# mazouziwissem/improving_yolov8_CBAM_SwinBlock

Hardware: AMD Instinct MI355X
Metric: images/sec fwd+bwd YOLOv8s-CBAM-Swin bs=32 640x640 (higher is better)
Workload: dtype bf16; 1 GPU; yolov8s.yaml (nc=1) forward + v8 loss + backward + clip + SGD-nesterov + EMA step, bs=32/GPU 640x640 (CBAM + 2x SwinBlock + SPPF5 + SPPF7); global_batch=32, imgsz=640, parallelism=dp1

## Files before the change

improving_yolov8_cbam_swinblock_amd/csrc/common.h:

```cpp
#pragma once
#include <hip/hip_runtime.h>
#include <stdint.h>
#include <stdio.h>

#include <type_traits>

#include "../../include/ymi.h"

typedef __bf16 bf16_t;
typedef __attribute__((ext_vector_type(8))) __bf16 bf16x8;
typedef __attribute__((ext_vector_type(4))) __bf16 bf16x4;
typedef __attribute__((ext_vector_type(4))) float f32x4;
typedef __attribute__((ext_vector_type(2))) float f32x2;
typedef __attribute__((ext_vector_type(4))) uint32_t u32x4;
typedef __attribute__((ext_vector_type(2))) uint32_t u32x2;

typedef const __attribute__((address_space(1))) void* gptr_t;
typedef __attribute__((address_space(3))) void* lptr_t;

#define YMI_WAVE 64

void ymi_set_error(const char* fmt, ...);
#define YMI_CHECK_ARG(cond, ...)          \
    do {                                  \
// ... 29 lines not shown
static inline bool ymi_same_shape(const ymi_tensor* a, const ymi_tensor* b) {
    return a->n == b->n && a->h == b->h && a->w == b->w && a->c == b->c;
}
enum YmiOpt {
    OPT_EW_PPT,
    OPT_EW_CAP,
    OPT_RED_CAP,
    OPT_XCD_SHIFT,
    OPT_ATTN_TILED,
    OPT_WGRAD_BLOCKS,
    OPT_WGRAD_BLOCKS128,
    OPT_IGEMM_TILE_BM,
    OPT_IGEMM_TILE_BN,
    OPT_BN_TAIL,
    OPT_WGRAD_PATCH,
    OPT_COUNT
};
int ymi_opt(int id);
static inline int ew_ppt() { return ymi_opt(OPT_EW_PPT); }
static inline int ew_cap() { return ymi_opt(OPT_EW_CAP); }
static inline int64_t ew_capped(int64_t gb) {
    if (gb > ew_cap()) gb = ew_cap();
    return (gb + 7) / 8 * 8;
}
static inline int64_t ew_blocks(int64_t P, int rows) {
    int64_t gb = (P + (int64_t)rows * ew_ppt() - 1) / ((int64_t)rows * ew_ppt());
    if (gb < 1024) gb = (P + rows - 1) / rows < 1024 ? (P + rows - 1) / rows : 1024;
    return ew_capped(gb);
}
template <typename T> struct TypeTag {
    typedef T type;
};
template <int ACT> using ActTag = std::integral_constant<int, ACT>;
// ... 411 lines not shown
```

improving_yolov8_cbam_swinblock_amd/csrc/runtime.hip:

```cpp
#include <stdarg.h>
#include <string.h>

#include <stdlib.h>

#include "common.h"

static thread_local char g_err[512] = "";

void ymi_set_error(const char* fmt, ...) {
    va_list ap;
    va_start(ap, fmt);
    vsnprintf(g_err, sizeof(g_err), fmt, ap);
    va_end(ap);
}

extern "C" int ymi_version(void) { return YMI_VERSION; }
extern "C" const char* ymi_last_error(void) { return g_err; }

__device__ __attribute__((aligned(256))) unsigned char ymi_zero_page_storage[256];

const void* ymi_zero_page() {
    static thread_local int cached_dev = -1;
    static thread_local void* cached_ptr = nullptr;
    int dev = 0;
// ... 1 lines not shown
    if (dev != cached_dev) {
        void* p = nullptr;
        if (hipGetSymbolAddress(&p, HIP_SYMBOL(ymi_zero_page_storage)) != hipSuccess) return nullptr;
        cached_ptr = p;
        cached_dev = dev;
    }
    return cached_ptr;
}

struct OptEntry {
    const char* name;
    int value;
};
static OptEntry g_opts[OPT_COUNT] = {
    {"ew_ppt", 64}, {"ew_cap", 512}, {"red_cap", 512}, {"xcd_shift", 0}, {"attn_tiled", 0}, {"wgrad_blocks", 1280}, {"wgrad_blocks128", 768},
    {"igemm_tile_bm", 0}, {"igemm_tile_bn", 0}, {"bn_tail", 0}, {"wgrad_patch", 1},
};
static void opts_from_env() {
    for (int i = 0; i < OPT_COUNT; ++i) {
        char env[64] = "YMI_";
        size_t n = 4;
        for (const char* c = g_opts[i].name; *c && n + 1 < sizeof(env); ++c) env[n++] = (char)((*c >= 'a' && *c <= 'z') ? *c - 32 : *c);
        env[n] = 0;
        if (const char* v = getenv(env)) g_opts[i].value = atoi(v);
    }
    if (const char* t = getenv("YMI_IGEMM_TILE")) {
        int bm = 0, bn = 0;
        if (sscanf(t, "%d,%d", &bm, &bn) == 2) {
            g_opts[OPT_IGEMM_TILE_BM].value = bm;
            g_opts[OPT_IGEMM_TILE_BN].value = bn;
        }
    }
}
int ymi_opt(int id) {
    static const bool init = (opts_from_env(), true);
    (void)init;
    return g_opts[id].value;
}
extern "C" int ymi_set_option(const char* name, int64_t value) {
    (void)ymi_opt(0);
    for (int i = 0; name && i < OPT_COUNT; ++i)
        if (!strcmp(name, g_opts[i].name)) {
            g_opts[i].value = (int)value;
            return YMI_OK;
        }
    ymi_set_error("set_option: unknown option '%s'", name ? name : "(null)");
    return YMI_EINVAL;
}
extern "C" int64_t ymi_get_option(const char* name) {
    (void)ymi_opt(0);
    for (int i = 0; name && i < OPT_COUNT; ++i)
        if (!strcmp(name, g_opts[i].name)) return g_opts[i].value;
// ... 22 lines not shown
```

improving_yolov8_cbam_swinblock_amd/csrc/wgrad.hip:

```cpp
#include <stdlib.h>

#include <mutex>
#include <type_traits>

#include "common.h"

struct WgradArgs {
    const void* x;
    const void* dy;
    void* slab;
    int slab_bf16;
    float* bias_slab;
    const void* zero;
    int64_t ldx, ldy;
    int Mpix, H, W, Ho, Wo;
    int stride, pad, KW;
    int CoutP, Cin, NG;
    int pix_per_split;
    int nx, ny, splits, xcd_map;
    int pw_shift;
    uint32_t x_bytes, y_bytes;
    uint32_t wo_mul, wo_shr, ho_mul, ho_shr;
};

__device__ __forceinline__ int wg_fast_div(int n, uint32_t mul, uint32_t shr) { return (int)((__umulhi((uint32_t)n, mul) + (uint32_t)n) >> shr); }

constexpr int WG_BN = 128;
constexpr int WG_BK = 32;
constexpr int WG_NS = 2;
constexpr int WG_WAVES = 5;

template <typename T, int BM> constexpr size_t wgrad_lds_bytes() { return (size_t)WG_NS * WG_BK * (BM + WG_BN) * sizeof(T); }

__device__ __forceinline__ void wg_buffer_to_lds(const void* base, uint32_t bytes, lptr_t dst, uint32_t voff, uint32_t soff) {
#if defined(__HIP_DEVICE_COMPILE__)
    __builtin_amdgcn_raw_ptr_buffer_load_lds(__builtin_amdgcn_make_buffer_rsrc(const_cast<void*>(base), 0, bytes, 0x00020000), dst, 16, voff, soff, 0, 0);
#endif
}
__device__ __forceinline__ void wg_global_to_lds(const void* src, lptr_t dst) {
#if defined(__HIP_DEVICE_COMPILE__)
    __builtin_amdgcn_global_load_lds((gptr_t)src, dst, 16, 0, 0);
#endif
}
template <typename T> struct WFrag;

template <> struct WFrag<bf16_t> {
    static __device__ __forceinline__ void read2(bf16x8& f, const TrFragAddr& ad) {
        typedef __attribute__((ext_vector_type(2))) uint32_t u2;
        u2 lo, hi;
        asm volatile("ds_read_b64_tr_b16 %0, %1" : "=v"(lo) : "v"((uint32_t)(uintptr_t)ad.lo));
        asm volatile("ds_read_b64_tr_b16 %0, %1" : "=v"(hi) : "v"((uint32_t)(uintptr_t)ad.hi));
        const u32x4 v = {lo[0], lo[1], hi[0], hi[1]};
        f = __builtin_bit_cast(bf16x8, v);
    }
    template <int BM, int TR, int TC, bool BIAS>
    static __device__ __forceinline__ void step(const char* Ys, const char* Xs, int r0, int c0, int lane, f32x4 (&acc)[TR][TC], bool bias, f32x4 (&accb)[BIAS ? TR : 1]) {
        static_assert(WG_BK == 32, "one 32-deep sub-step");
        bf16x8 af[TR], bfr[TC];
        TrFragAddr ay[TR], ax[TC];
#pragma unroll
        for (int t = 0; t < TR; ++t) ay[t] = tr_frag_addr<tr_swz_mode(BM * 2)>(Ys, BM * 2, r0 + t * 16, lane);
#pragma unroll
        for (int t = 0; t < TC; ++t) ax[t] = tr_frag_addr<tr_swz_mode(WG_BN * 2)>(Xs, WG_BN * 2, c0 + t * 16, lane);
        __builtin_amdgcn_sched_barrier(0);
#pragma unroll
        for (int t = 0; t < TC; ++t) read2(bfr[t], ax[t]);
#pragma unroll
        for (int t = 0; t < TR; ++t) read2(af[t], ay[t]);
#pragma unroll
        for (int a = 0; a < TR; ++a) {
            __builtin_amdgcn_sched_barrier(0);
            if (a == 0) asm volatile("s_waitcnt lgkmcnt(%0)" ::"n"(2 * (TR - 1)) : "memory");
            else if (a == 1) asm volatile("s_waitcnt lgkmcnt(%0)" ::"n"(TR > 2 ? 2 * (TR - 2) : 0) : "memory");
            else if (a == 2) asm volatile("s_waitcnt lgkmcnt(%0)" ::"n"(TR > 3 ? 2 * (TR - 3) : 0) : "memory");
            else asm volatile("s_waitcnt lgkmcnt(0)" ::: "memory");
            asm volatile("" : "+v"(af[a]));
            if (a == 0) {
#pragma unroll
// ... 1 lines not shown
            }
#pragma unroll
            for (int b = 0; b < TC; ++b)
                acc[a][b] = __builtin_amdgcn_mfma_f32_16x16x32_bf16(bfr[b], af[a], acc[a][b], 0, 0, 0);
            if (BIAS && bias) {
                typedef __attribute__((ext_vector_type(8))) short s16x8;
                const s16x8 one8 = {0x3F80, 0x3F80, 0x3F80, 0x3F80, 0x3F80, 0x3F80, 0x3F80, 0x3F80};
                const bf16x8 ones = __builtin_bit_cast(bf16x8, one8);
                if constexpr (BIAS) accb[a] = __builtin_amdgcn_mfma_f32_16x16x32_bf16(ones, af[a], accb[a], 0, 0, 0);
            }
        }
        __builtin_amdgcn_sched_barrier(0);
    }
};
template <> struct WFrag<float> {
    template <int BM, int TR, int TC, bool BIAS>
    static __device__ __forceinline__ void step(const char* Ys, const char* Xs, int r0, int c0, int lane, f32x4 (&acc)[TR][TC], bool bias, f32x4 (&accb)[BIAS ? TR : 1]) {
        const int kq = lane >> 4, i = lane & 15;
#pragma unroll
        for (int ks = 0; ks < WG_BK / 4; ++ks) {
            float af[TR], bfr[TC];
#pragma unroll
            for (int t = 0; t < TR; ++t) af[t] = *reinterpret_cast<const float*>(Ys + ((4 * ks + kq) * BM + r0 + t * 16 + i) * 4);
#pragma unroll
            for (int t = 0; t < TC; ++t) bfr[t] = *reinterpret_cast<const float*>(Xs + ((4 * ks + kq) * WG_BN + c0 + t * 16 + i) * 4);
#pragma unroll
            for (int a = 0; a < TR; ++a)
#pragma unroll
                for (int b = 0; b < TC; ++b) acc[a][b] = __builtin_amdgcn_mfma_f32_16x16x4f32(bfr[b], af[a], acc[a][b], 0, 0, 0);
            if (BIAS && bias) {
#pragma unroll
                for (int a = 0; a < (BIAS ? TR : 1); ++a) accb[a] = __builtin_amdgcn_mfma_f32_16x16x4f32(1.0f, af[a], accb[a], 0, 0, 0);
            }
        }
    }
};

template <typename T, int BM> struct WgTile {
    static constexpr int NT = 256;
    static constexpr int CH = ElemTraits<T>::CH, ES = (int)sizeof(T);
    static constexpr int YCW = BM * ES / 16, XCW = WG_BN * ES / 16;
    static constexpr int YT = WG_BK * YCW < NT ? WG_BK * YCW : NT;
    static constexpr int NY = (WG_BK * YCW + NT - 1) / NT, NX = WG_BK * XCW / NT;
    static constexpr int WCOLS = WG_BN / 64, WROWS = (NT / 64) / WCOLS;
    static constexpr int WM = BM / WROWS, TR = WM / 16, TC = 4;
    static constexpr int YBYTES = WG_BK * BM * ES, XBYTES = WG_BK * WG_BN * ES, STAGE = YBYTES + XBYTES;
    static_assert(NY >= 1 && NX >= 1, "tile too small");
    static constexpr bool SWZ = std::is_same<T, bf16_t>::value;
    static_assert(NT / XCW >= 16 || !SWZ, "bf16: a block-wide load covers >= 16 rows, so a thread's rows share the row bits the swizzle uses");
    int yrow0, ych;
    bool y_cok, x_cok;
    int xrow0, ci, dh, dw;
    __device__ __forceinline__ WgTile(const WgradArgs& a, int tid, int j0, int co0) {
        const int ytid = tid % YT;
        yrow0 = ytid / YCW;
        const int ycc = SWZ ? ((ytid % YCW) ^ (tr_swz<tr_swz_mode(YCW * 16)>(yrow0) << 1)) : (ytid % YCW);
        ych = co0 + ycc * CH;
        y_cok = ych < a.CoutP;
        xrow0 = tid / XCW;
        const int xcc = SWZ ? ((tid % XCW) ^ (tr_swz<tr_swz_mode(XCW * 16)>(xrow0) << 1)) : (tid % XCW);
        const int j = j0 + xcc * CH;
        x_cok = j < a.NG;
        const int tap = x_cok ? j / a.Cin : 0;
        ci = x_cok ? j - tap * a.Cin : 0;
        dh = tap / a.KW - a.pad;
        dw = tap % a.KW - a.pad;
    }
    __device__ __forceinline__ int y_row(int i) const { return yrow0 + i * (NT / YCW); }
    __device__ __forceinline__ int x_row(int i) const { return xrow0 + i * (NT / XCW); }
    static __device__ __forceinline__ lptr_t y_slot(char* Ys, int i, int wave) { return (lptr_t)(Ys + (i * NT + (wave * 64) % YT) * 16); }
    static __device__ __forceinline__ lptr_t x_slot(char* Xs, int i, int wave) { return (lptr_t)(Xs + (i * NT + wave * 64) * 16); }
};

template <typename T, int BM> struct WgRasterWalk {
    using G = WgTile<T, BM>;
    const WgradArgs& a;
    const G& ld;
    const int wave, m_end;
    const int s_ = a.stride, ldx32 = (int)a.ldx, ldy32 = (int)a.ldy;
    const int q_ = WG_BK / a.Wo, r_ = WG_BK - q_ * a.Wo;
    const uint32_t d_step = (uint32_t)((q_ * s_ * a.W + r_ * s_) * ldx32);
    const uint32_t d_wwrap = (uint32_t)((s_ * a.W - a.Wo * s_) * ldx32);
    const uint32_t d_hwrap = (uint32_t)((a.H * a.W - a.Ho * s_ * a.W) * ldx32);
    const uint32_t y_step = (uint32_t)(WG_BK * ldy32);
    const int ws_lim = a.Wo * s_, hs_lim = a.Ho * s_;
    int x_ws[G::NX], x_hs[G::NX];
    uint32_t x_off[G::NX], y_off[G::NY];
    __device__ __forceinline__ WgRasterWalk(const WgradArgs& a_, const G& ld_, int wave_, int m_begin)
        : a(a_), ld(ld_), wave(wave_), m_end(min(a_.Mpix, m_begin + a_.pix_per_split)) {
#pragma unroll
        for (int i = 0; i < G::NX; ++i) {
            const int m = m_begin + ld.x_row(i);
            const int t = wg_fast_div(m, a.wo_mul, a.wo_shr);
            const int wo = m - t * a.Wo;
            const int n = wg_fast_div(t, a.ho_mul, a.ho_shr);
            const int ho = t - n * a.Ho;
            x_ws[i] = wo * s_;
            x_hs[i] = ho * s_;
            x_off[i] = (uint32_t)(((n * a.H + ho * s_ + ld.dh) * a.W + wo * s_ + ld.dw) * ldx32 + ld.ci);
        }
#pragma unroll
        for (int i = 0; i < G::NY; ++i) y_off[i] = (uint32_t)((m_begin + ld.y_row(i)) * ldy32 + ld.ych);
    }
    __device__ __forceinline__ void issue(char* Ys, int mk) {
        const T* __restrict__ xg = reinterpret_cast<const T*>(a.x);
        const T* __restrict__ yg = reinterpret_cast<const T*>(a.dy);
        const T* zero = reinterpret_cast<const T*>(a.zero);
        char* Xs = Ys + G::YBYTES;
        const int left = m_end - mk;
#pragma unroll
        for (int i = 0; i < G::NY; ++i) {
            const bool ok = ld.y_cok && ld.y_row(i) < left;
            const T* src = ok ? yg + y_off[i] : zero;
            wg_global_to_lds(src, ld.y_slot(Ys, i, wave));
            y_off[i] += y_step;
        }
#pragma unroll
        for (int i = 0; i < G::NX; ++i) {
            const bool ok = ld.x_cok && ld.x_row(i) < left && (unsigned)(x_hs[i] + ld.dh) < (unsigned)a.H && (unsigned)(x_ws[i] + ld.dw) < (unsigned)a.W;
            const T* src = ok ? xg + x_off[i] : zero;
            wg_global_to_lds(src, ld.x_slot(Xs, i, wave));
            x_ws[i] += r_ * s_;
            x_hs[i] += q_ * s_;
            x_off[i] += d_step;
            if (x_ws[i] >= ws_lim) {
                x_ws[i] -= ws_lim;
                x_hs[i] += s_;
                x_off[i] += d_wwrap;
            }
            while (x_hs[i] >= hs_lim) {
                x_hs[i] -= hs_lim;
                x_off[i] += d_hwrap;
            }
        }
    }
};

template <typename T, int BM> struct WgPatchWalk {
    using G = WgTile<T, BM>;
    static constexpr uint32_t OOR = 0x80000000u;
    static constexpr int ES = G::ES;
    const WgradArgs& a;
    const int wave;
    const int s_ = a.stride, ldx32 = (int)a.ldx, ldy32 = (int)a.ldy;
    const int pw = 1 << a.pw_shift, ph = WG_BK >> a.pw_shift;
    const uint32_t xbias = (uint32_t)((a.W + 1) * ldx32 * ES);
    uint32_t pvx[G::NX], pvy[G::NY];
    int pch[G::NX], pcw[G::NX];
    int p_wo, p_ho;
    uint32_t p_sx, p_sy;
    __device__ __forceinline__ WgPatchWalk(const WgradArgs& a_, const G& ld, int wave_, int m_begin) : a(a_), wave(wave_) {
#pragma unroll
        for (int i = 0; i < G::NX; ++i) {
            const int row = ld.x_row(i);
            const int pr = row >> a.pw_shift, pc = row & (pw - 1);
            pch[i] = pr * s_ + ld.dh;
            pcw[i] = pc * s_ + ld.dw;
            pvx[i] = ld.x_cok ? (uint32_t)(((pch[i] * a.W + pcw[i]) * ldx32 + ld.ci) * ES) + xbias : OOR;
        }
#pragma unroll
        for (int i = 0; i < G::NY; ++i) {
            const int row = ld.y_row(i);
            const int pr = row >> a.pw_shift, pc = row & (pw - 1);
            pvy[i] = ld.y_cok ? (uint32_t)(((pr * a.Wo + pc) * ldy32 + ld.ych) * ES) : OOR;
        }
        const int pidx = __builtin_amdgcn_readfirstlane(m_begin / WG_BK);
        const int npw = a.Wo >> a.pw_shift, nph = a.Ho / ph;
        const int t = pidx / npw, wp = pidx - t * npw;
        const int n = t / nph, hp = t - n * nph;
        p_wo = wp * pw;
        p_ho = hp * ph;
        p_sx = (uint32_t)(((n * a.H + p_ho * s_) * a.W + p_wo * s_) * ldx32 * ES);
        p_sy = (uint32_t)(((n * a.Ho + p_ho) * a.Wo + p_wo) * ldy32 * ES);
// ... 14 lines not shown
        p_sx += (uint32_t)(pw * s_ * ldx32 * ES);
        p_sy += (uint32_t)(pw * ldy32 * ES);
        if (p_wo == a.Wo) {
            p_wo = 0;
            p_ho += ph;
            p_sx += (uint32_t)((ph * s_ * a.W - a.Wo * s_) * ldx32 * ES);
            p_sy += (uint32_t)((ph * a.Wo - a.Wo) * ldy32 * ES);
            if (p_ho == a.Ho) {
                p_ho = 0;
                p_sx += (uint32_t)((a.H * a.W - a.Ho * s_ * a.W) * ldx32 * ES);
            }
        }
    }
};

template <typename S, int TR> struct SlabStage {
    static constexpr int ES = (int)sizeof(S);
    static constexpr int SROW = 64 * ES + 16;
    static constexpr int CPR = 64 * ES / 16;
    static constexpr int RPI = 64 / CPR;
    static constexpr int RP = TR < 4 / ES ? TR : 4 / ES;
    static constexpr int BYTES = RP * 16 * SROW;
    static_assert(TR % RP == 0, "whole passes");
};
template <typename S, int TR, int TC>
__device__ __forceinline__ void wg_store_slab_staged(char* ring, int wave, int lane, const f32x4 (&acc)[TR][TC], S* slab, int row0, int col0, int CoutP, int NG) {
    using St = SlabStage<S, TR>;
    constexpr int ES = St::ES, SROW = St::SROW, RP = St::RP;
    static_assert(TC * 16 == 64, "a wave's tile is 64 columns wide");
    __syncthreads();
    asm volatile("" : "+v"(lane));
    char* st = ring + wave * St::BYTES;
    const int l15 = lane & 15, l4 = lane >> 4;
    const int srow = lane / St::CPR, sch = lane % St::CPR;
    const int col = col0 + sch * (16 / ES);
#pragma unroll
    for (int r0 = 0; r0 < TR; r0 += RP) {
#pragma unroll
        for (int rr = 0; rr < RP; ++rr)
#pragma unroll
            for (int c = 0; c < TC; ++c) {
                char* p = st + (rr * 16 + l15) * SROW + (c * 16 + 4 * l4) * ES;
                if constexpr (std::is_same<S, float>::value) {
                    *reinterpret_cast<f32x4*>(p) = acc[r0 + rr][c];
                } else {
                    const bf16x4 v = {(bf16_t)acc[r0 + rr][c][0], (bf16_t)acc[r0 + rr][c][1], (bf16_t)acc[r0 + rr][c][2], (bf16_t)acc[r0 + rr][c][3]};
                    *reinterpret_cast<bf16x4*>(p) = v;
                }
            }
        __builtin_amdgcn_fence(__ATOMIC_RELEASE, "wavefront");
        __builtin_amdgcn_wave_barrier();
        __builtin_amdgcn_fence(__ATOMIC_ACQUIRE, "wavefront");
#pragma unroll
        for (int k = 0; k < RP * 16 / St::RPI; ++k) {
            const int row = k * St::RPI + srow;
            const u32x4 u = *reinterpret_cast<const u32x4*>(st + row * SROW + sch * 16);
            const int co = row0 + r0 * 16 + row;
            if (co < CoutP && col < NG) *reinterpret_cast<u32x4*>(slab + (int64_t)co * NG + col) = u;
        }
        __builtin_amdgcn_fence(__ATOMIC_RELEASE, "wavefront");
        __builtin_amdgcn_wave_barrier();
        __builtin_amdgcn_fence(__ATOMIC_ACQUIRE, "wavefront");
    }
}

template <typename T, int BM, bool BIAS, bool PATCH>
__global__ __launch_bounds__(256, (BM == 128 ? 3 : WG_WAVES)) void wgrad_kernel(WgradArgs a, BnRider rider) {
    using G = WgTile<T, BM>;
    constexpr int NT = G::NT, TR = G::TR, TC = G::TC, WM = G::WM, STAGE = G::STAGE, NS = WG_NS;
    constexpr int LDS = (int)wgrad_lds_bytes<T, BM>();
    static_assert(LDS == NS * STAGE, "the launcher's LDS bytes are the ring");
    static_assert(LDS >= (NT / 64) * SlabStage<bf16_t, TR>::BYTES && LDS >= (NT / 64) * SlabStage<float, TR>::BYTES, "the staged slab stores use the ring");
    static_assert(LDS >= BN_FINAL_RED * (int)sizeof(double), "a rider workgroup sums its slices in the ring");
    extern __shared__ __attribute__((aligned(16))) char smem[];

    const int tid = threadIdx.x, lane = tid & 63;
    const int wave = __builtin_amdgcn_readfirstlane(tid >> 6);
    const int wr = wave / G::WCOLS, wc = wave % G::WCOLS;
    int bx, by, bz;
    if (rider.nwg && (int)blockIdx.x < rider.nwg) {
        if ((int)blockIdx.x * 32 < rider.f.C) bn_final_block<NT, false>(rider.f, (int)blockIdx.x, reinterpret_cast<double*>(smem));
        return;
    }
    if (a.xcd_map) {
        const int id = (int)blockIdx.x - rider.nwg, xcd = id & 7, seq = id >> 3, nxy = a.nx * a.ny;
        const int zi = seq / nxy, t = seq - zi * nxy;
        const int spx = (a.splits + 7) >> 3;
        bz = xcd * spx + zi;
        if (zi >= spx || bz >= a.splits) return;
        by = t / a.nx;
        bx = t - by * a.nx;
    } else {
        bx = blockIdx.x; by = blockIdx.y; bz = blockIdx.z;
    }
    const int j0 = bx * WG_BN, co0 = by * BM;
    const int m_begin = bz * a.pix_per_split;
    const int m_end = min(a.Mpix, m_begin + a.pix_per_split);
    const G ld(a, tid, j0, co0);
    typename std::conditional<PATCH, WgPatchWalk<T, BM>, WgRasterWalk<T, BM>>::type walk(a, ld, wave, m_begin);

    f32x4 acc[TR][TC];
#pragma unroll
    for (int r = 0; r < TR; ++r)
#pragma unroll
        for (int c = 0; c < TC; ++c) acc[r][c] = f32x4{0.f, 0.f, 0.f, 0.f};

    const bool do_bias = BIAS && bx == 0 && wc == 0;
    f32x4 accb[BIAS ? TR : 1];
#pragma unroll
    for (int r = 0; r < (BIAS ? TR : 1); ++r) accb[r] = f32x4{0.f, 0.f, 0.f, 0.f};
    const int nk = (m_end - m_begin + WG_BK - 1) / WG_BK;
    constexpr int LPT = G::NY + G::NX;
#pragma unroll
    for (int s = 0; s < NS - 1; ++s)
        if (s < nk) walk.issue(smem + s * STAGE, m_begin + s * WG_BK);
    for (int kt = 0; kt < nk; ++kt) {
        if (kt + NS - 2 < nk) wait_vmcnt_barrier<LPT * (NS - 2)>();
        else wait_vmcnt_barrier<0>();
        if (kt + NS - 1 < nk) walk.issue(smem + ((kt + NS - 1) % NS) * STAGE, m_begin + (kt + NS - 1) * WG_BK);
        const char* Ys = smem + (kt % NS) * STAGE;
        WFrag<T>::template step<BM, TR, TC, BIAS>(Ys, Ys + G::YBYTES, wr * WM, wc * 64, lane, acc, do_bias, accb);
    }

    const int64_t slab_off = (int64_t)bz * a.CoutP * a.NG;
    const int row0 = co0 + wr * WM, col0 = j0 + wc * 64;
    const int l15 = lane & 15, l4 = lane >> 4;
    if (BIAS && do_bias && l4 == 0) {
#pragma unroll
        for (int r = 0; r < (BIAS ? TR : 1); ++r) {
            const int co = row0 + r * 16 + l15;
            if (co < a.CoutP) a.bias_slab[(int64_t)bz * a.CoutP + co] = accb[r][0];
        }
    }
    if constexpr (std::is_same<T, bf16_t>::value) {
        if (a.slab_bf16) wg_store_slab_staged<bf16_t>(smem, wave, lane, acc, reinterpret_cast<bf16_t*>(a.slab) + slab_off, row0, col0, a.CoutP, a.NG);
        else wg_store_slab_staged<float>(smem, wave, lane, acc, reinterpret_cast<float*>(a.slab) + slab_off, row0, col0, a.CoutP, a.NG);
    } else {
#pragma unroll
        for (int r = 0; r < TR; ++r) {
            const int co = row0 + r * 16 + l15;
// ... 98 lines not shown
        if (tab[mid].first_block <= (int)blockIdx.x) lo = mid;
        else hi = mid - 1;
    }
    const ymi_wgrad_pending e = tab[lo];
    if (e.slab_bf16) reduce_batch_body<true>(e, red);
    else reduce_batch_body<false>(e, red);
}

static void wg_find_divisor(int d, uint32_t* mul, uint32_t* shr) {
    int lg = 0;
    while ((1 << lg) < d) ++lg;
    *mul = (uint32_t)((((uint64_t)1 << 32) * (((uint64_t)1 << lg) - (uint64_t)d)) / (uint64_t)d + 1);
    *shr = (uint32_t)lg;
}

struct WgradPlan {
    int splits, pix_per_split;
    size_t slab_bytes;
};
static int wgrad_bm(int64_t coutp, bool bf16) {
    if (!bf16) return 64;
    if (coutp <= 32) return 32;
    return (coutp >= 128 && coutp % 128 == 0) || coutp >= 256 ? 128 : 64;
}
static WgradPlan wgrad_plan(int64_t mpix, int64_t coutp, int64_t ng, int bm, size_t slab_esize) {
    const int64_t tiles = ((ng + WG_BN - 1) / WG_BN) * ((coutp + bm - 1) / bm);
    const int target64 = ymi_opt(OPT_WGRAD_BLOCKS);
    const int target128 = ymi_opt(OPT_WGRAD_BLOCKS128);
    const int target = bm == 128 ? target128 : target64;
    int64_t s = (target + tiles - 1) / tiles;
    const int64_t smax = (mpix + 255) / 256;
    if (s > smax) s = smax;
    if (s < 1) s = 1;
    if (s >= 8) s = (s + 7) / 8 * 8 <= smax ? (s + 7) / 8 * 8 : s / 8 * 8;
    int64_t pps = (mpix + s - 1) / s;
    pps = (pps + WG_BK - 1) / WG_BK * WG_BK;
    s = (mpix + pps - 1) / pps;
    WgradPlan p;
    p.splits = (int)s;
    p.pix_per_split = (int)pps;
    p.slab_bytes = ((size_t)s * coutp * ng * slab_esize + 255) / 256 * 256;
    return p;
}

static int64_t pad_to(int64_t v, int64_t m) { return (v + m - 1) / m * m; }
constexpr int64_t WG_BIAS_ROWS = 2048 * 2 + 1;

extern "C" size_t ymi_conv2d_bwd_weight_workspace(int64_t m_rows, int64_t cout, int64_t cin, int64_t kh, int64_t kw) {
    const int64_t coutp = pad_to(cout, 8), cinp = pad_to(cin, 8);
    WgradPlan p = wgrad_plan(m_rows, coutp, kh * kw * cinp, 64, 4);
    const WgradPlan p128 = wgrad_plan(m_rows, coutp, kh * kw * cinp, 128, 4);
    if (p128.slab_bytes > p.slab_bytes) p = p128;
    return p.slab_bytes + (size_t)WG_BIAS_ROWS * coutp * sizeof(float) + 256;
}

static int wgrad_impl(const ymi_tensor* x, const ymi_tensor* dy, int64_t cout_real, int64_t cin_real, int64_t kh, int64_t kw, int64_t stride,
                      float* dw_oihw, float* dbias, void* workspace, size_t workspace_bytes, ymi_wgrad_pending* pending, void* stream);

struct WgradLaunch {
    WgradArgs a;
    dim3 grid;
    int bm;
    bool bf16;
    hipStream_t s;
    double flop, bytes;
};
template <typename T, int BM> static void wgrad_launch_tile(const WgradArgs& a, const BnRider& r, dim3 grid, hipStream_t s) {
    constexpr size_t lds = wgrad_lds_bytes<T, BM>();
    static_assert(lds <= 64 * 1024, "a larger ring needs hipFuncAttributeMaxDynamicSharedMemorySize");
    void (*kernel)(WgradArgs, BnRider) = a.bias_slab ? wgrad_kernel<T, BM, true, false> : wgrad_kernel<T, BM, false, false>;
    if constexpr (std::is_same<T, bf16_t>::value) {
        if (a.pw_shift >= 0) kernel = a.bias_slab ? wgrad_kernel<T, BM, true, true> : wgrad_kernel<T, BM, false, true>;
    }
    hipLaunchKernelGGL(kernel, grid, dim3(256), lds, s, a, r);
}
static void wgrad_launch(const WgradLaunch& h, const BnFinal* rider) {
    BnRider r{};
    dim3 grid = h.grid;
    if (rider && h.a.xcd_map) {
        r.f = *rider;
        r.nwg = ((rider->C + 31) / 32 + 7) / 8 * 8;
        grid.x += (unsigned)r.nwg;
    }
    int prof = -1;
    if (ymi_prof_enabled()) prof = ymi_prof_start(h.s, 1, h.flop, h.bytes, h.bf16 ? 2500.0 : 157.3);
    if (!h.bf16) wgrad_launch_tile<float, 64>(h.a, r, grid, h.s);
    else if (h.bm == 128) wgrad_launch_tile<bf16_t, 128>(h.a, r, grid, h.s);
    else if (h.bm == 32) wgrad_launch_tile<bf16_t, 32>(h.a, r, grid, h.s);
    else wgrad_launch_tile<bf16_t, 64>(h.a, r, grid, h.s);
    ymi_prof_stop(h.s, prof);
}
static struct WgradHeld {
    std::mutex mu;
    bool on = false;
    bool valid = false;
    WgradLaunch launch;
    int device = 0;
} g_held;
static int wgrad_current_device() {
    int d = 0;
    (void)hipGetDevice(&d);
// ... 83 lines not shown

static int wgrad_impl(const ymi_tensor* x, const ymi_tensor* dy, int64_t cout_real, int64_t cin_real, int64_t kh, int64_t kw, int64_t stride,
                      float* dw_oihw, float* dbias, void* workspace, size_t workspace_bytes, ymi_wgrad_pending* pending, void* stream) {
    YMI_CHECK_ARG(ymi_tensor_ok(x) && ymi_tensor_ok(dy) && dw_oihw && workspace, "conv2d_bwd_weight: bad argument");
    YMI_CHECK_ARG(x->dtype == dy->dtype, "conv2d_bwd_weight: dtype mismatch");
    const int ch = x->dtype == YMI_BF16 ? 8 : 4;
    YMI_CHECK_ARG(x->c % ch == 0 && x->ld % ch == 0 && dy->c % ch == 0 && dy->ld % ch == 0, "conv2d_bwd_weight: channels must be multiples of %d", ch);
    YMI_CHECK_ARG(kh == kw && (kh == 1 || kh == 3) && (stride == 1 || stride == 2), "conv2d_bwd_weight: k in {1,3}, stride in {1,2}");
    const int64_t pad = kh / 2;
    YMI_CHECK_ARG(dy->n == x->n && dy->h == (x->h + 2 * pad - kh) / stride + 1 && dy->w == (x->w + 2 * pad - kw) / stride + 1, "conv2d_bwd_weight: shapes");
    YMI_CHECK_ARG(cout_real <= dy->c && cin_real <= x->c, "conv2d_bwd_weight: real channel counts");
    YMI_CHECK_ARG(ymi_pixels(x) * x->ld < (1ll << 31) && ymi_pixels(dy) * dy->ld < (1ll << 31), "conv2d_bwd_weight: too large");
    const int64_t mpix = ymi_pixels(dy);
    const int64_t ng = kh * kw * x->c;
    const bool bf16 = x->dtype == YMI_BF16;
    const int bm = wgrad_bm(dy->c, bf16), bn = WG_BN;
    WgradPlan p = wgrad_plan(mpix, dy->c, ng, bm, bf16 ? 2 : 4);
    const bool slab_bf16 = bf16 && p.splits >= 16;
    if (bf16 && !slab_bf16) p = wgrad_plan(mpix, dy->c, ng, bm, 4);
    size_t need = p.slab_bytes + (dbias ? (size_t)WG_BIAS_ROWS * dy->c * sizeof(float) : 0);
    if (workspace_bytes < need) {
        ymi_set_error("conv2d_bwd_weight: workspace %zu < %zu bytes", workspace_bytes, need);
        return YMI_EWORKSPACE;
    }
    WgradArgs a{};
    a.x = x->data; a.dy = dy->data; a.slab = workspace; a.slab_bf16 = slab_bf16 ? 1 : 0; a.zero = ymi_zero_page();
    a.bias_slab = dbias ? reinterpret_cast<float*>(reinterpret_cast<char*>(workspace) + p.slab_bytes) : nullptr;
    YMI_CHECK_ARG(!dbias || p.splits <= WG_BIAS_ROWS, "conv2d_bwd_weight: too many splits for the bias partials");
    a.ldx = x->ld; a.ldy = dy->ld;
    a.Mpix = (int)mpix; a.H = (int)x->h; a.W = (int)x->w; a.Ho = (int)dy->h; a.Wo = (int)dy->w;
    a.stride = (int)stride; a.pad = (int)pad; a.KW = (int)kw;
    a.CoutP = (int)dy->c; a.Cin = (int)x->c; a.NG = (int)ng; a.pix_per_split = p.pix_per_split;
    wg_find_divisor(a.Wo, &a.wo_mul, &a.wo_shr);
    wg_find_divisor(a.Ho, &a.ho_mul, &a.ho_shr);
// ... 7 lines not shown
                const int pw = 1 << sh, ph = WG_BK >> sh;
                if (dy->w % pw == 0 && dy->h % ph == 0) {
                    a.pw_shift = sh;
                    break;
                }
            }
            a.x_bytes = (uint32_t)xb;
            a.y_bytes = (uint32_t)yb;
        }
    }
    a.xcd_map = p.splits >= 8 ? 1 : 0;
    dim3 grid((unsigned)a.nx, (unsigned)a.ny, (unsigned)p.splits);
    if (a.xcd_map) grid = dim3((unsigned)(8 * ((p.splits + 7) / 8) * a.nx * a.ny), 1, 1);
    hipStream_t s = (hipStream_t)stream;
    const double es = (double)ymi_esize(x->dtype);
    WgradLaunch h{a, grid, bm, bf16, s, 2.0 * (double)mpix * (double)dy->c * (double)ng,
                  ((double)ymi_pixels(x) * x->c + (double)mpix * dy->c) * es + (double)dy->c * ng * 4.0};
    {
        std::lock_guard<std::mutex> lk(g_held.mu);
        wgrad_flush_held_locked();
        if (pending && g_held.on && a.xcd_map) {
            g_held.launch = h;
            g_held.device = wgrad_current_device();
            g_held.valid = true;
        } else {
            wgrad_launch(h, nullptr);
        }
    }
    YMI_CHECK_LAUNCH("wgrad");
    if (pending) {
        *pending = ymi_wgrad_record(a.slab, dw_oihw, (int64_t)a.CoutP * a.NG, p.splits, a.NG, a.Cin, (int)cout_real, (int)cin_real, (int)(kh * kw), slab_bf16,
// ... 16 lines not shown
```

Baseline: 2791 images/sec.

## Add shape-matched wgrad tile widths for narrow 1x1 and 3x3 Cin=32 convs

Adds two new bf16 weight-gradient tile forms: a 64-wide N tile for 1x1 convs with at most 64 input channels, and a 288-wide tile built from nine 32-channel tap sub-images for 3x3 convs with Cin=32. This avoids wasted MFMA work and padded loads when the reduction dimension (taps*Cin) does not fill 128-column tiles. The change brings a wide-tile MFMA step with grouped LDS reads, generalised slab staging, and occupancy-aware split planning. The risks are more register and LDS pressure for the 288 tile and more template instantiations.

```diff
diff --git a/improving_yolov8_cbam_swinblock_amd/csrc/common.h b/improving_yolov8_cbam_swinblock_amd/csrc/common.h
--- a/improving_yolov8_cbam_swinblock_amd/csrc/common.h
+++ b/improving_yolov8_cbam_swinblock_amd/csrc/common.h
@@ -67,9 +67,12 @@
     OPT_IGEMM_TILE_BN,
     OPT_BN_TAIL,
     OPT_WGRAD_PATCH,
+    OPT_WGRAD_BN,
+    OPT_WGRAD_BN_LAST,
     OPT_COUNT
 };
 int ymi_opt(int id);
+void ymi_opt_store(int id, int value);
 static inline int ew_ppt() { return ymi_opt(OPT_EW_PPT); }
 static inline int ew_cap() { return ymi_opt(OPT_EW_CAP); }
 static inline int64_t ew_capped(int64_t gb) {
diff --git a/improving_yolov8_cbam_swinblock_amd/csrc/runtime.hip b/improving_yolov8_cbam_swinblock_amd/csrc/runtime.hip
--- a/improving_yolov8_cbam_swinblock_amd/csrc/runtime.hip
+++ b/improving_yolov8_cbam_swinblock_amd/csrc/runtime.hip
@@ -39,7 +39,7 @@
 };
 static OptEntry g_opts[OPT_COUNT] = {
     {"ew_ppt", 64}, {"ew_cap", 512}, {"red_cap", 512}, {"xcd_shift", 0}, {"attn_tiled", 0}, {"wgrad_blocks", 1280}, {"wgrad_blocks128", 768},
-    {"igemm_tile_bm", 0}, {"igemm_tile_bn", 0}, {"bn_tail", 0}, {"wgrad_patch", 1},
+    {"igemm_tile_bm", 0}, {"igemm_tile_bn", 0}, {"bn_tail", 0}, {"wgrad_patch", 1}, {"wgrad_bn", 0}, {"wgrad_bn_last", 0},
 };
 static void opts_from_env() {
     for (int i = 0; i < OPT_COUNT; ++i) {
@@ -61,6 +61,10 @@
     static const bool init = (opts_from_env(), true);
     (void)init;
     return g_opts[id].value;
+}
+void ymi_opt_store(int id, int value) {
+    (void)ymi_opt(0);
+    g_opts[id].value = value;
 }
 extern "C" int ymi_set_option(const char* name, int64_t value) {
     (void)ymi_opt(0);
diff --git a/improving_yolov8_cbam_swinblock_amd/csrc/wgrad.hip b/improving_yolov8_cbam_swinblock_amd/csrc/wgrad.hip
--- a/improving_yolov8_cbam_swinblock_amd/csrc/wgrad.hip
+++ b/improving_yolov8_cbam_swinblock_amd/csrc/wgrad.hip
@@ -30,7 +30,14 @@
 constexpr int WG_NS = 2;
 constexpr int WG_WAVES = 5;
 
-template <typename T, int BM> constexpr size_t wgrad_lds_bytes() { return (size_t)WG_NS * WG_BK * (BM + WG_BN) * sizeof(T); }
+constexpr size_t WG_LDS_MIN = 4 * 16 * (64 * 4 + 16);
+template <typename T, int BM, int BN = WG_BN> constexpr size_t wgrad_lds_bytes() {
+    return (size_t)WG_NS * WG_BK * (BM + BN) * sizeof(T) > WG_LDS_MIN ? (size_t)WG_NS * WG_BK * (BM + BN) * sizeof(T) : WG_LDS_MIN;
+}
+template <typename T, int BM, int BN> constexpr int wgrad_min_waves() {
+    const int by_lds = (int)(160 * 1024 / wgrad_lds_bytes<T, BM, BN>()), by_regs = BM == 128 ? 3 : WG_WAVES;
+    return BN <= WG_BN || by_regs < by_lds ? by_regs : by_lds;
+}
 
 __device__ __forceinline__ void wg_buffer_to_lds(const void* base, uint32_t bytes, lptr_t dst, uint32_t voff, uint32_t soff) {
 #if defined(__HIP_DEVICE_COMPILE__)
@@ -53,15 +60,73 @@
         const u32x4 v = {lo[0], lo[1], hi[0], hi[1]};
         f = __builtin_bit_cast(bf16x8, v);
     }
-    template <int BM, int TR, int TC, bool BIAS>
+    template <int BN, int SUB> static __device__ __forceinline__ TrFragAddr x_addr(const char* Xs, int c, int lane) {
+        if constexpr (SUB == BN) {
+            return tr_frag_addr<tr_swz_mode(BN * 2)>(Xs, BN * 2, c, lane);
+        } else {
+            const int sub = c / SUB;
+            return tr_frag_addr<tr_swz_mode(SUB * 2)>(Xs + sub * (WG_BK * SUB * 2), SUB * 2, c - sub * SUB, lane);
+        }
+    }
+    template <int BM, int BN, int SUB, int TR, int TC, bool BIAS>
+    static __device__ __forceinline__ void step_wide(const char* Ys, const char* Xs, int r0, int c0, int lane, f32x4 (&acc)[TR][TC], bool bias, f32x4 (&accb)[BIAS ? TR : 1]) {
+        constexpr int GS = TC % 3 == 0 ? 3 : 2, NGR = TC / GS;
+        static_assert(TC % GS == 0, "whole groups");
+        bf16x8 af[TR], bfr[2][GS];
+        TrFragAddr ay[TR], ax[GS];
+#pragma unroll
+        for (int t = 0; t < TR; ++t) ay[t] = tr_frag_addr<tr_swz_mode(BM * 2)>(Ys, BM * 2, r0 + t * 16, lane);
+#pragma unroll
+        for (int t = 0; t < GS; ++t) ax[t] = x_addr<BN, SUB>(Xs, c0 + t * 16, lane);
+        __builtin_amdgcn_sched_barrier(0);
+#pragma unroll
+        for (int t = 0; t < TR; ++t) read2(af[t], ay[t]);
+#pragma unroll
+        for (int t = 0; t < GS; ++t) read2(bfr[0][t], ax[t]);
+#pragma unroll
+        for (int g = 0; g < NGR; ++g) {
+            if (g + 1 < NGR) {
+#pragma unroll
+                for (int t = 0; t < GS; ++t) ax[t] = x_addr<BN, SUB>(Xs, c0 + ((g + 1) * GS + t) * 16, lane);
+                __builtin_amdgcn_sched_barrier(0);
+#pragma unroll
+                for (int t = 0; t < GS; ++t) read2(bfr[(g + 1) & 1][t], ax[t]);
+                asm volatile("s_waitcnt lgkmcnt(%0)" ::"n"(2 * GS) : "memory");
+            } else {
+                __builtin_amdgcn_sched_barrier(0);
+                asm volatile("s_waitcnt lgkmcnt(0)" ::: "memory");
+            }
+            if (g == 0) {
+#pragma unroll
+                for (int a = 0; a < TR; ++a) asm volatile("" : "+v"(af[a]));
+            }
+#pragma unroll
+            for (int b = 0; b < GS; ++b) asm volatile("" : "+v"(bfr[g & 1][b]));
+#pragma unroll
+            for (int a = 0; a < TR; ++a) {
+#pragma unroll
+                for (int b = 0; b < GS; ++b)
+                    acc[a][g * GS + b] = __builtin_amdgcn_mfma_f32_16x16x32_bf16(bfr[g & 1][b], af[a], acc[a][g * GS + b], 0, 0, 0);
+                if (BIAS && bias && g == 0) {
+                    typedef __attribute__((ext_vector_type(8))) short s16x8;
+                    const s16x8 one8 = {0x3F80, 0x3F80, 0x3F80, 0x3F80, 0x3F80, 0x3F80, 0x3F80, 0x3F80};
+                    const bf16x8 ones = __builtin_bit_cast(bf16x8, one8);
+                    if constexpr (BIAS) accb[a] = __builtin_amdgcn_mfma_f32_16x16x32_bf16(ones, af[a], accb[a], 0, 0, 0);
+                }
+            }
+            __builtin_amdgcn_sched_barrier(0);
+        }
+    }
+    template <int BM, int BN, int SUB, int TR, int TC, bool BIAS>
     static __device__ __forceinline__ void step(const char* Ys, const char* Xs, int r0, int c0, int lane, f32x4 (&acc)[TR][TC], bool bias, f32x4 (&accb)[BIAS ? TR : 1]) {
         static_assert(WG_BK == 32, "one 32-deep sub-step");
+        if constexpr (TC > 4) return step_wide<BM, BN, SUB, TR, TC, BIAS>(Ys, Xs, r0, c0, lane, acc, bias, accb);
         bf16x8 af[TR], bfr[TC];
         TrFragAddr ay[TR], ax[TC];
 #pragma unroll
         for (int t = 0; t < TR; ++t) ay[t] = tr_frag_addr<tr_swz_mode(BM * 2)>(Ys, BM * 2, r0 + t * 16, lane);
 #pragma unroll
-        for (int t = 0; t < TC; ++t) ax[t] = tr_frag_addr<tr_swz_mode(WG_BN * 2)>(Xs, WG_BN * 2, c0 + t * 16, lane);
+        for (int t = 0; t < TC; ++t) ax[t] = x_addr<BN, SUB>(Xs, c0 + t * 16, lane);
         __builtin_amdgcn_sched_barrier(0);
 #pragma unroll
         for (int t = 0; t < TC; ++t) read2(bfr[t], ax[t]);
@@ -93,8 +158,9 @@
     }
 };
 template <> struct WFrag<float> {
-    template <int BM, int TR, int TC, bool BIAS>
+    template <int BM, int BN, int SUB, int TR, int TC, bool BIAS>
     static __device__ __forceinline__ void step(const char* Ys, const char* Xs, int r0, int c0, int lane, f32x4 (&acc)[TR][TC], bool bias, f32x4 (&accb)[BIAS ? TR : 1]) {
+        static_assert(SUB == BN, "parity mode: one X image");
         const int kq = lane >> 4, i = lane & 15;
 #pragma unroll
         for (int ks = 0; ks < WG_BK / 4; ++ks) {
@@ -102,7 +168,7 @@
 #pragma unroll
             for (int t = 0; t < TR; ++t) af[t] = *reinterpret_cast<const float*>(Ys + ((4 * ks + kq) * BM + r0 + t * 16 + i) * 4);
 #pragma unroll
-            for (int t = 0; t < TC; ++t) bfr[t] = *reinterpret_cast<const float*>(Xs + ((4 * ks + kq) * WG_BN + c0 + t * 16 + i) * 4);
+            for (int t = 0; t < TC; ++t) bfr[t] = *reinterpret_cast<const float*>(Xs + ((4 * ks + kq) * BN + c0 + t * 16 + i) * 4);
 #pragma unroll
             for (int a = 0; a < TR; ++a)
 #pragma unroll
@@ -115,44 +181,69 @@
     }
 };
 
-template <typename T, int BM> struct WgTile {
+template <typename T, int BM, int BN = WG_BN, int SUB = BN> struct WgTile {
     static constexpr int NT = 256;
     static constexpr int CH = ElemTraits<T>::CH, ES = (int)sizeof(T);
-    static constexpr int YCW = BM * ES / 16, XCW = WG_BN * ES / 16;
+    static constexpr bool TAPF = SUB != BN;
+    static constexpr int YCW = BM * ES / 16, XCW = SUB * ES / 16;
+    static constexpr int XP = WG_BK * BN * ES / 16, XSP = WG_BK * XCW;
     static constexpr int YT = WG_BK * YCW < NT ? WG_BK * YCW : NT;
-    static constexpr int NY = (WG_BK * YCW + NT - 1) / NT, NX = WG_BK * XCW / NT;
-    static constexpr int WCOLS = WG_BN / 64, WROWS = (NT / 64) / WCOLS;
-    static constexpr int WM = BM / WROWS, TR = WM / 16, TC = 4;
-    static constexpr int YBYTES = WG_BK * BM * ES, XBYTES = WG_BK * WG_BN * ES, STAGE = YBYTES + XBYTES;
-    static_assert(NY >= 1 && NX >= 1, "tile too small");
+    static constexpr int NY = (WG_BK * YCW + NT - 1) / NT, NX = (XP + NT - 1) / NT;
+    static constexpr int XTL = XP - (NX - 1) * NT;
+    static constexpr int WCOLS = BN >= 128 ? 2 : 1, WROWS = (NT / 64) / WCOLS;
+    static constexpr int WM = BM / WROWS, WN = BN / WCOLS, TR = WM / 16, TC = WN / 16;
+    static constexpr int YBYTES = WG_BK * BM * ES, XBYTES = WG_BK * BN * ES, STAGE = YBYTES + XBYTES;
+    static_assert(NY >= 1 && NX >= 1 && TR >= 1 && WM % 16 == 0 && WN % 16 == 0 && BN % SUB == 0, "tile too small");
+    static_assert(XTL % 64 == 0 && NT % XTL == 0, "the last X load is whole waves; the others repeat it");
+    static_assert(!TAPF || (NT % XSP == 0 && XTL % XSP == 0), "whole-tap form: a block-wide load is whole sub-images, so a thread keeps its row");
     static constexpr bool SWZ = std::is_same<T, bf16_t>::value;
-    static_assert(NT / XCW >= 16 || !SWZ, "bf16: a block-wide load covers >= 16 rows, so a thread's rows share the row bits the swizzle uses");
+    static_assert((TAPF ? XSP : NT) / XCW >= 16 || !SWZ, "bf16: a block-wide load covers >= 16 rows, so a thread's rows share the row bits the swizzle uses");
     int yrow0, ych;
     bool y_cok, x_cok;
     int xrow0, ci, dh, dw;
+    int tap0, tapl, ntap;
     __device__ __forceinline__ WgTile(const WgradArgs& a, int tid, int j0, int co0) {
         const int ytid = tid % YT;
         yrow0 = ytid / YCW;
         const int ycc = SWZ ? ((ytid % YCW) ^ (tr_swz<tr_swz_mode(YCW * 16)>(yrow0) << 1)) : (ytid % YCW);
         ych = co0 + ycc * CH;
         y_cok = ych < a.CoutP;
-        xrow0 = tid / XCW;
-        const int xcc = SWZ ? ((tid % XCW) ^ (tr_swz<tr_swz_mode(XCW * 16)>(xrow0) << 1)) : (tid % XCW);
-        const int j = j0 + xcc * CH;
-        x_cok = j < a.NG;
-        const int tap = x_cok ? j / a.Cin : 0;
-        ci = x_cok ? j - tap * a.Cin : 0;
-        dh = tap / a.KW - a.pad;
-        dw = tap % a.KW - a.pad;
+        if constexpr (TAPF) {
+            xrow0 = (tid % XSP) / XCW;
+            const int xcc = SWZ ? ((tid % XCW) ^ (tr_swz<tr_swz_mode(XCW * 16)>(xrow0) << 1)) : (tid % XCW);
+            ci = xcc * CH;
+            x_cok = true;
+            dh = dw = 0;
+            tap0 = j0 / SUB + tid / XSP;
+            tapl = j0 / SUB + (NX - 1) * (NT / XSP) + (tid % XTL) / XSP;
+            ntap = a.KW * a.KW;
+        } else {
+            xrow0 = tid / XCW;
+            const int xcc = SWZ ? ((tid % XCW) ^ (tr_swz<tr_swz_mode(XCW * 16)>(xrow0) << 1)) : (tid % XCW);
+            const int j = j0 + xcc * CH;
+            x_cok = j < a.NG;
+            const int tap = x_cok ? j / a.Cin : 0;
+            ci = x_cok ? j - tap * a.Cin : 0;
+            dh = tap / a.KW - a.pad;
+            dw = tap % a.KW - a.pad;
+            tap0 = tapl = ntap = 0;
+        }
     }
     __device__ __forceinline__ int y_row(int i) const { return yrow0 + i * (NT / YCW); }
-    __device__ __forceinline__ int x_row(int i) const { return xrow0 + i * (NT / XCW); }
+    __device__ __forceinline__ int x_row(int i) const { return TAPF ? xrow0 : xrow0 + i * (NT / XCW); }
+    __device__ __forceinline__ int x_tap(int i) const { return i == NX - 1 ? tapl : tap0 + i * (NT / XSP); }
+    __device__ __forceinline__ bool x_ok(int i) const { return TAPF ? x_tap(i) < ntap : x_cok; }
+    __device__ __forceinline__ int x_dh(int i) const { return TAPF ? x_tap(i) / 3 - 1 : dh; }
+    __device__ __forceinline__ int x_dw(int i) const { return TAPF ? x_tap(i) % 3 - 1 : dw; }
     static __device__ __forceinline__ lptr_t y_slot(char* Ys, int i, int wave) { return (lptr_t)(Ys + (i * NT + (wave * 64) % YT) * 16); }
-    static __device__ __forceinline__ lptr_t x_slot(char* Xs, int i, int wave) { return (lptr_t)(Xs + (i * NT + wave * 64) * 16); }
-};
-
-template <typename T, int BM> struct WgRasterWalk {
-    using G = WgTile<T, BM>;
+    static __device__ __forceinline__ lptr_t x_slot(char* Xs, int i, int wave) {
+        if constexpr (XTL == NT) return (lptr_t)(Xs + (i * NT + wave * 64) * 16);
+        else return (lptr_t)(Xs + (i * NT + (i == NX - 1 ? (wave * 64) % XTL : wave * 64)) * 16);
+    }
+};
+
+template <typename T, int BM, int BN = WG_BN, int SUB = BN> struct WgRasterWalk {
+    using G = WgTile<T, BM, BN, SUB>;
     const WgradArgs& a;
     const G& ld;
     const int wave, m_end;
@@ -176,7 +267,7 @@
             const int ho = t - n * a.Ho;
             x_ws[i] = wo * s_;
             x_hs[i] = ho * s_;
-            x_off[i] = (uint32_t)(((n * a.H + ho * s_ + ld.dh) * a.W + wo * s_ + ld.dw) * ldx32 + ld.ci);
+            x_off[i] = (uint32_t)(((n * a.H + ho * s_ + ld.x_dh(i)) * a.W + wo * s_ + ld.x_dw(i)) * ldx32 + ld.ci);
         }
 #pragma unroll
         for (int i = 0; i < G::NY; ++i) y_off[i] = (uint32_t)((m_begin + ld.y_row(i)) * ldy32 + ld.ych);
@@ -196,7 +287,7 @@
         }
 #pragma unroll
         for (int i = 0; i < G::NX; ++i) {
-            const bool ok = ld.x_cok && ld.x_row(i) < left && (unsigned)(x_hs[i] + ld.dh) < (unsigned)a.H && (unsigned)(x_ws[i] + ld.dw) < (unsigned)a.W;
+            const bool ok = ld.x_ok(i) && ld.x_row(i) < left && (unsigned)(x_hs[i] + ld.x_dh(i)) < (unsigned)a.H && (unsigned)(x_ws[i] + ld.x_dw(i)) < (unsigned)a.W;
             const T* src = ok ? xg + x_off[i] : zero;
             wg_global_to_lds(src, ld.x_slot(Xs, i, wave));
             x_ws[i] += r_ * s_;
@@ -215,8 +306,8 @@
     }
 };
 
-template <typename T, int BM> struct WgPatchWalk {
-    using G = WgTile<T, BM>;
+template <typename T, int BM, int BN = WG_BN, int SUB = BN> struct WgPatchWalk {
+    using G = WgTile<T, BM, BN, SUB>;
     static constexpr uint32_t OOR = 0x80000000u;
     static constexpr int ES = G::ES;
     const WgradArgs& a;
@@ -233,9 +324,9 @@
         for (int i = 0; i < G::NX; ++i) {
             const int row = ld.x_row(i);
             const int pr = row >> a.pw_shift, pc = row & (pw - 1);
-            pch[i] = pr * s_ + ld.dh;
-            pcw[i] = pc * s_ + ld.dw;
-            pvx[i] = ld.x_cok ? (uint32_t)(((pch[i] * a.W + pcw[i]) * ldx32 + ld.ci) * ES) + xbias : OOR;
+            pch[i] = pr * s_ + ld.x_dh(i);
+            pcw[i] = pc * s_ + ld.x_dw(i);
+            pvx[i] = ld.x_ok(i) ? (uint32_t)(((pch[i] * a.W + pcw[i]) * ldx32 + ld.ci) * ES) + xbias : OOR;
         }
 #pragma unroll
         for (int i = 0; i < G::NY; ++i) {
@@ -280,10 +371,10 @@
     }
 };
 
-template <typename S, int TR> struct SlabStage {
+template <typename S, int TR, int WN = 64> struct SlabStage {
     static constexpr int ES = (int)sizeof(S);
-    static constexpr int SROW = 64 * ES + 16;
-    static constexpr int CPR = 64 * ES / 16;
+    static constexpr int SROW = WN * ES + 16;
+    static constexpr int CPR = WN * ES / 16;
     static constexpr int RPI = 64 / CPR;
     static constexpr int RP = TR < 4 / ES ? TR : 4 / ES;
     static constexpr int BYTES = RP * 16 * SROW;
@@ -291,9 +382,8 @@
 };
 template <typename S, int TR, int TC>
 __device__ __forceinline__ void wg_store_slab_staged(char* ring, int wave, int lane, const f32x4 (&acc)[TR][TC], S* slab, int row0, int col0, int CoutP, int NG) {
-    using St = SlabStage<S, TR>;
+    using St = SlabStage<S, TR, TC * 16>;
     constexpr int ES = St::ES, SROW = St::SROW, RP = St::RP;
-    static_assert(TC * 16 == 64, "a wave's tile is 64 columns wide");
     __syncthreads();
     asm volatile("" : "+v"(lane));
     char* st = ring + wave * St::BYTES;
@@ -317,12 +407,22 @@
         __builtin_amdgcn_fence(__ATOMIC_RELEASE, "wavefront");
         __builtin_amdgcn_wave_barrier();
         __builtin_amdgcn_fence(__ATOMIC_ACQUIRE, "wavefront");
-#pragma unroll
-        for (int k = 0; k < RP * 16 / St::RPI; ++k) {
-            const int row = k * St::RPI + srow;
-            const u32x4 u = *reinterpret_cast<const u32x4*>(st + row * SROW + sch * 16);
-            const int co = row0 + r0 * 16 + row;
-            if (co < CoutP && col < NG) *reinterpret_cast<u32x4*>(slab + (int64_t)co * NG + col) = u;
+        if constexpr (64 % St::CPR == 0) {
+#pragma unroll
+            for (int k = 0; k < RP * 16 / St::RPI; ++k) {
+                const int row = k * St::RPI + srow;
+                const u32x4 u = *reinterpret_cast<const u32x4*>(st + row * SROW + sch * 16);
+                const int co = row0 + r0 * 16 + row;
+                if (co < CoutP && col < NG) *reinterpret_cast<u32x4*>(slab + (int64_t)co * NG + col) = u;
+            }
+        } else {
+#pragma unroll
+            for (int k = 0; k < (RP * 16 * St::CPR + 63) / 64; ++k) {
+                const int idx = k * 64 + lane, row = idx / St::CPR, ch = idx - row * St::CPR;
+                const int co = row0 + r0 * 16 + row, cc = col0 + ch * (16 / ES);
+                if (idx < RP * 16 * St::CPR && co < CoutP && cc < NG)
+                    *reinterpret_cast<u32x4*>(slab + (int64_t)co * NG + cc) = *reinterpret_cast<const u32x4*>(st + row * SROW + ch * 16);
+            }
         }
         __builtin_amdgcn_fence(__ATOMIC_RELEASE, "wavefront");
         __builtin_amdgcn_wave_barrier();
@@ -330,13 +430,13 @@
     }
 }
 
-template <typename T, int BM, bool BIAS, bool PATCH>
-__global__ __launch_bounds__(256, (BM == 128 ? 3 : WG_WAVES)) void wgrad_kernel(WgradArgs a, BnRider rider) {
-    using G = WgTile<T, BM>;
-    constexpr int NT = G::NT, TR = G::TR, TC = G::TC, WM = G::WM, STAGE = G::STAGE, NS = WG_NS;
-    constexpr int LDS = (int)wgrad_lds_bytes<T, BM>();
-    static_assert(LDS == NS * STAGE, "the launcher's LDS bytes are the ring");
-    static_assert(LDS >= (NT / 64) * SlabStage<bf16_t, TR>::BYTES && LDS >= (NT / 64) * SlabStage<float, TR>::BYTES, "the staged slab stores use the ring");
+template <typename T, int BM, bool BIAS, bool PATCH, int BN = WG_BN, int SUB = BN>
+__global__ __launch_bounds__(256, (wgrad_min_waves<T, BM, BN>())) void wgrad_kernel(WgradArgs a, BnRider rider) {
+    using G = WgTile<T, BM, BN, SUB>;
+    constexpr int NT = G::NT, TR = G::TR, TC = G::TC, WM = G::WM, WN = G::WN, STAGE = G::STAGE, NS = WG_NS;
+    constexpr int LDS = (int)wgrad_lds_bytes<T, BM, BN>();
+    static_assert(LDS >= NS * STAGE, "the launcher's LDS bytes hold the ring");
+    static_assert(LDS >= (NT / 64) * SlabStage<bf16_t, TR, WN>::BYTES && LDS >= (NT / 64) * SlabStage<float, TR, WN>::BYTES, "the staged slab stores use the ring");
     static_assert(LDS >= BN_FINAL_RED * (int)sizeof(double), "a rider workgroup sums its slices in the ring");
     extern __shared__ __attribute__((aligned(16))) char smem[];
 
@@ -359,11 +459,11 @@
     } else {
         bx = blockIdx.x; by = blockIdx.y; bz = blockIdx.z;
     }
-    const int j0 = bx * WG_BN, co0 = by * BM;
+    const int j0 = bx * BN, co0 = by * BM;
     const int m_begin = bz * a.pix_per_split;
     const int m_end = min(a.Mpix, m_begin + a.pix_per_split);
     const G ld(a, tid, j0, co0);
-    typename std::conditional<PATCH, WgPatchWalk<T, BM>, WgRasterWalk<T, BM>>::type walk(a, ld, wave, m_begin);
+    typename std::conditional<PATCH, WgPatchWalk<T, BM, BN, SUB>, WgRasterWalk<T, BM, BN, SUB>>::type walk(a, ld, wave, m_begin);
 
     f32x4 acc[TR][TC];
 #pragma unroll
@@ -385,11 +485,11 @@
         else wait_vmcnt_barrier<0>();
         if (kt + NS - 1 < nk) walk.issue(smem + ((kt + NS - 1) % NS) * STAGE, m_begin + (kt + NS - 1) * WG_BK);
         const char* Ys = smem + (kt % NS) * STAGE;
-        WFrag<T>::template step<BM, TR, TC, BIAS>(Ys, Ys + G::YBYTES, wr * WM, wc * 64, lane, acc, do_bias, accb);
+        WFrag<T>::template step<BM, BN, SUB, TR, TC, BIAS>(Ys, Ys + G::YBYTES, wr * WM, wc * WN, lane, acc, do_bias, accb);
     }
 
     const int64_t slab_off = (int64_t)bz * a.CoutP * a.NG;
-    const int row0 = co0 + wr * WM, col0 = j0 + wc * 64;
+    const int row0 = co0 + wr * WM, col0 = j0 + wc * WN;
     const int l15 = lane & 15, l4 = lane >> 4;
     if (BIAS && do_bias && l4 == 0) {
 #pragma unroll
@@ -518,6 +618,7 @@
     *shr = (uint32_t)lg;
 }
 
+static int64_t pad_to(int64_t v, int64_t m) { return (v + m - 1) / m * m; }
 struct WgradPlan {
     int splits, pix_per_split;
     size_t slab_bytes;
@@ -527,11 +628,23 @@
     if (coutp <= 32) return 32;
     return (coutp >= 128 && coutp % 128 == 0) || coutp >= 256 ? 128 : 64;
 }
-static WgradPlan wgrad_plan(int64_t mpix, int64_t coutp, int64_t ng, int bm, size_t slab_esize) {
-    const int64_t tiles = ((ng + WG_BN - 1) / WG_BN) * ((coutp + bm - 1) / bm);
+struct WgradForm {
+    int bm, bn, sub;
+};
+static WgradForm wgrad_form(int64_t coutp, int64_t cinp, int64_t taps, bool bf16, int opt_bn) {
+    const int bm = wgrad_bm(coutp, bf16);
+    WgradForm f{bm, WG_BN, WG_BN};
+    if (!bf16 || bm == 128 || opt_bn == WG_BN) return f;
+    if (taps == 1 && cinp <= 64 && bm == 64) f.bn = f.sub = 64;
+    else if (taps == 9 && cinp == 32 && bm == 64) f.bn = 288, f.sub = 32;
+    return f;
+}
+static WgradPlan wgrad_plan(int64_t mpix, int64_t coutp, int64_t ng, int bm, size_t slab_esize, int bn = WG_BN) {
+    const int64_t tiles = ((ng + bn - 1) / bn) * ((coutp + bm - 1) / bm);
     const int target64 = ymi_opt(OPT_WGRAD_BLOCKS);
     const int target128 = ymi_opt(OPT_WGRAD_BLOCKS128);
-    const int target = bm == 128 ? target128 : target64;
+    const int per_cu = bn == 288 ? wgrad_min_waves<bf16_t, 64, 288>() : WG_WAVES;
+    const int target = bm == 128 ? target128 : target64 * per_cu / WG_WAVES;
     int64_t s = (target + tiles - 1) / tiles;
     const int64_t smax = (mpix + 255) / 256;
     if (s > smax) s = smax;
@@ -547,7 +660,6 @@
     return p;
 }
 
-static int64_t pad_to(int64_t v, int64_t m) { return (v + m - 1) / m * m; }
 constexpr int64_t WG_BIAS_ROWS = 2048 * 2 + 1;
 
 extern "C" size_t ymi_conv2d_bwd_weight_workspace(int64_t m_rows, int64_t cout, int64_t cin, int64_t kh, int64_t kw) {
@@ -555,6 +667,9 @@
     WgradPlan p = wgrad_plan(m_rows, coutp, kh * kw * cinp, 64, 4);
     const WgradPlan p128 = wgrad_plan(m_rows, coutp, kh * kw * cinp, 128, 4);
     if (p128.slab_bytes > p.slab_bytes) p = p128;
+    const WgradForm f = wgrad_form(coutp, cinp, kh * kw, true, 0);
+    const WgradPlan pf = wgrad_plan(m_rows, coutp, kh * kw * cinp, f.bm, 4, f.bn);
+    if (pf.slab_bytes > p.slab_bytes) p = pf;
     return p.slab_bytes + (size_t)WG_BIAS_ROWS * coutp * sizeof(float) + 256;
 }
 
@@ -564,17 +679,17 @@
 struct WgradLaunch {
     WgradArgs a;
     dim3 grid;
-    int bm;
+    int bm, bn;
     bool bf16;
     hipStream_t s;
     double flop, bytes;
 };
-template <typename T, int BM> static void wgrad_launch_tile(const WgradArgs& a, const BnRider& r, dim3 grid, hipStream_t s) {
-    constexpr size_t lds = wgrad_lds_bytes<T, BM>();
+template <typename T, int BM, int BN = WG_BN, int SUB = BN> static void wgrad_launch_tile(const WgradArgs& a, const BnRider& r, dim3 grid, hipStream_t s) {
+    constexpr size_t lds = wgrad_lds_bytes<T, BM, BN>();
     static_assert(lds <= 64 * 1024, "a larger ring needs hipFuncAttributeMaxDynamicSharedMemorySize");
-    void (*kernel)(WgradArgs, BnRider) = a.bias_slab ? wgrad_kernel<T, BM, true, false> : wgrad_kernel<T, BM, false, false>;
+    void (*kernel)(WgradArgs, BnRider) = a.bias_slab ? wgrad_kernel<T, BM, true, false, BN, SUB> : wgrad_kernel<T, BM, false, false, BN, SUB>;
     if constexpr (std::is_same<T, bf16_t>::value) {
-        if (a.pw_shift >= 0) kernel = a.bias_slab ? wgrad_kernel<T, BM, true, true> : wgrad_kernel<T, BM, false, true>;
+        if (a.pw_shift >= 0) kernel = a.bias_slab ? wgrad_kernel<T, BM, true, true, BN, SUB> : wgrad_kernel<T, BM, false, true, BN, SUB>;
     }
     hipLaunchKernelGGL(kernel, grid, dim3(256), lds, s, a, r);
 }
@@ -589,6 +704,8 @@
     int prof = -1;
     if (ymi_prof_enabled()) prof = ymi_prof_start(h.s, 1, h.flop, h.bytes, h.bf16 ? 2500.0 : 157.3);
     if (!h.bf16) wgrad_launch_tile<float, 64>(h.a, r, grid, h.s);
+    else if (h.bn == 64) wgrad_launch_tile<bf16_t, 64, 64>(h.a, r, grid, h.s);
+    else if (h.bn == 288) wgrad_launch_tile<bf16_t, 64, 288, 32>(h.a, r, grid, h.s);
     else if (h.bm == 128) wgrad_launch_tile<bf16_t, 128>(h.a, r, grid, h.s);
     else if (h.bm == 32) wgrad_launch_tile<bf16_t, 32>(h.a, r, grid, h.s);
     else wgrad_launch_tile<bf16_t, 64>(h.a, r, grid, h.s);
@@ -702,10 +819,12 @@
     const int64_t mpix = ymi_pixels(dy);
     const int64_t ng = kh * kw * x->c;
     const bool bf16 = x->dtype == YMI_BF16;
-    const int bm = wgrad_bm(dy->c, bf16), bn = WG_BN;
-    WgradPlan p = wgrad_plan(mpix, dy->c, ng, bm, bf16 ? 2 : 4);
+    const WgradForm form = wgrad_form(dy->c, x->c, kh * kw, bf16, ymi_opt(OPT_WGRAD_BN));
+    const int bm = form.bm, bn = form.bn;
+    ymi_opt_store(OPT_WGRAD_BN_LAST, bn);
+    WgradPlan p = wgrad_plan(mpix, dy->c, ng, bm, bf16 ? 2 : 4, bn);
     const bool slab_bf16 = bf16 && p.splits >= 16;
-    if (bf16 && !slab_bf16) p = wgrad_plan(mpix, dy->c, ng, bm, 4);
+    if (bf16 && !slab_bf16) p = wgrad_plan(mpix, dy->c, ng, bm, 4, bn);
     size_t need = p.slab_bytes + (dbias ? (size_t)WG_BIAS_ROWS * dy->c * sizeof(float) : 0);
     if (workspace_bytes < need) {
         ymi_set_error("conv2d_bwd_weight: workspace %zu < %zu bytes", workspace_bytes, need);
@@ -743,7 +862,7 @@
     if (a.xcd_map) grid = dim3((unsigned)(8 * ((p.splits + 7) / 8) * a.nx * a.ny), 1, 1);
     hipStream_t s = (hipStream_t)stream;
     const double es = (double)ymi_esize(x->dtype);
-    WgradLaunch h{a, grid, bm, bf16, s, 2.0 * (double)mpix * (double)dy->c * (double)ng,
+    WgradLaunch h{a, grid, bm, bn, bf16, s, 2.0 * (double)mpix * (double)dy->c * (double)ng,
                   ((double)ymi_pixels(x) * x->c + (double)mpix * dy->c) * es + (double)dy->c * ng * 4.0};
     {
         std::lock_guard<std::mutex> lk(g_held.mu);
```

After: 2796 images/sec (median of 5 runs). No clear change (+0.2%).
